# Meng-333/SRADSGAN

Hardware: AMD Instinct MI355X
Metric: training images/sec (216x216, x4) (higher is better)
Workload: dtype f32 (split-bf16 products: 3 bf16 MFMA terms per fp32 multiply, fp32 accumulate)

## Files before the change

sradsgan_amd/csrc/conv_api.hip:

```cpp
#include "conv_internal.h"
#include "conv_dev.h"

using namespace srhip;

namespace srhip {
struct PackEntry {
  const float* w;
  float* packed;
  int cout, cin, kh, kw, mode, fast;
};
__global__ __launch_bounds__(256) void pack_batched_kernel(const PackEntry* __restrict__ tab) {
  const PackEntry e = tab[blockIdx.y];
  const int khkw = e.kh * e.kw;
  if (e.fast) {
    constexpr int LDS_F = 32 * (16 * 9 + 1);
    __shared__ float tile[LDS_F];
    const long total = (long)e.cout * e.cin * khkw;
    const int RO = e.mode == 0 ? 8 : 32;
    const int CI = e.mode == 0 ? (khkw <= 9 ? 64 : 16) : (khkw <= 9 ? 16 : 4);
    const int ld = CI * khkw + 1;
    const int nci = (e.cin + CI - 1) / CI, nco = (e.cout + RO - 1) / RO;
    const int ndst = e.mode == 0 ? e.cout : e.cin, csrc = e.mode == 0 ? e.cin : e.cout;
    const long ndst16 = ((long)ndst + 15) / 16 * 16;
    float* s0 = e.packed;
// ... 194 lines not shown
  }
  if (key == 12) {
    g_flat_blocks = value > 0 ? value : 768;
    return SRHIP_OK;
  }
  if (key == 13) {
    g_flat_abl = value;
    return SRHIP_OK;
  }
  if (key == 14) {
    g_flat_f32_k8 = value;
    return SRHIP_OK;
  }
  if (key == 15) {
    g_patch8 = value;
    return SRHIP_OK;
  }
  if (key == 16) {
    g_patch8_abl = value;
    return SRHIP_OK;
  }
  if (key == 17) {
    g_phase_batch = value;
    return SRHIP_OK;
  }
  if (key == 18) {
    g_headconv_rows = value;
    return SRHIP_OK;
  }
  if (key == 19) {
    g_pool_epi_any = value;
    return SRHIP_OK;
  }
  return SRHIP_ERR_ARG;
}

int srhip_set_conv_math(int mode) {
  SRHIP_REQUIRE(mode == SRHIP_MATH_FP32 || mode == SRHIP_MATH_BF16X3 || mode == SRHIP_MATH_HALF, "set_conv_math: unknown mode");
  g_conv_math = mode;
  return SRHIP_OK;
}
int srhip_get_conv_math(void) { return g_conv_math; }

size_t srhip_packed_elems(int cout, int cin, int kh, int kw, int mode) {
  if (cout <= 0 || cin <= 0 || kh <= 0 || kw <= 0 || (mode != 0 && mode != 1)) return 0;
  const bool fast = mode == 0 ? fast_fwd_ok(cin, cout, kh, kw) : fast_dgrad_ok(cin, cout, kh, kw);
  if (fast)
    return 3 * (size_t)cout * cin * kh * kw + (size_t)fast_tiled_elems(mode == 0 ? cout : cin, mode == 0 ? cin : cout, kh * kw);
  const int csrc = mode == 0 ? cin : cout, cdst = mode == 0 ? cout : cin;
  return (size_t)kh * kw * csrc * legacy_packed_ld(cdst);
}

int srhip_pack_entry_bytes(void) { return (int)sizeof(PackEntry); }

int srhip_packed_is_fast(int cout, int cin, int kh, int kw, int mode) {
  return (mode == 0 ? fast_fwd_ok(cin, cout, kh, kw) : fast_dgrad_ok(cin, cout, kh, kw)) ? 1 : 0;
}

int srhip_pack_weights_batched(const void* entries_dev, int count, void* stream) {
  SRHIP_REQUIRE(entries_dev && count >= 0, "pack_weights_batched: bad argument");
  if (count == 0) return SRHIP_OK;
  hipLaunchKernelGGL(pack_batched_kernel, dim3(32, count), dim3(256), 0, as_stream(stream),
                     static_cast<const PackEntry*>(entries_dev));
  return check_launch("pack_weights_batched");
}

// ... 327 lines not shown
```

sradsgan_amd/csrc/conv_fast.hip:

```cpp
#include "conv_dev.h"

namespace srhip {

int g_fast_ablate = 0;



template <int BM, int BN, int WM, int WN, int BK, int MATH = 0>
__global__ __launch_bounds__(WM* WN * 64) void fast_conv_kernel(const float* __restrict__ src,
                                                                 const float* __restrict__ wt,
                                                                 const float* __restrict__ bias,
                                                                 const float* __restrict__ residual,
                                                                 const float* __restrict__ rowscale,
                                                                 const float* __restrict__ chanscale,
                                                                 const float* __restrict__ actmask,
                                                                 float* __restrict__ dst, FastGeom g, int nblk_m,
                                                                 int nblk_n) {
  constexpr int NT = WM * WN * 64;
  constexpr int WTM = BM / WM, WTN = BN / WN;
  constexpr int TM = WTM / 32, TN = WTN / 32;
  constexpr int LS = BK + 4;
  constexpr int QPR = BK / 4;
  constexpr int RPP = NT / QPR;
  constexpr int AR = (BM + RPP - 1) / RPP, BR = (BN + RPP - 1) / RPP;
// ... 2740 lines not shown
  if (g_conv_math >= 1 && g_wgrad_cfg == 0 && p.bn == 64 && cout % 256 == 0) p.bm = 256;
  if (rowtap == 1) { p.bm = 128; p.bn = 192; }
  if (rowtap == 2) { p.bm = 64; p.bn = 384; }
  const long tiles = (long)cdiv(cout, p.bm) * cdiv(ktot, p.bn);
  const int nchunks = cdiv(P, p.bk);
  const long target = rowtap ? (g_wgrad_cfg >= 100 ? g_wgrad_cfg : 768) : 640;
  long ns = (target + tiles - 1) / tiles;
  const long maxsplit = (nchunks + 15) / 16;
  if (ns > maxsplit) ns = maxsplit;
  if (ns > (tiles <= 2 ? 768 : 256)) ns = tiles <= 2 ? 768 : 256;
  if (ns < 1) ns = 1;
  if (ns >= 8) ns = (ns + 7) / 8 * 8;
  p.chunks_per_split = (int)((nchunks + ns - 1) / ns);
  p.nsplit = cdiv(nchunks, p.chunks_per_split);
  if (p.nsplit >= 8 && p.nsplit % 8 != 0) p.nsplit = (p.nsplit + 7) / 8 * 8;
  return p;
}

static int tail1x1_splits_per_image(int n, int hw) {
  int sp = cdiv(256, n);
  if (sp > cdiv(hw, 64)) sp = cdiv(hw, 64);
  return sp < 1 ? 1 : sp;
}
size_t fast_conv2d_wgrad_workspace(int n, int h, int w, int cin, int cout, int kh, int kw, int stride, int pad) {
  const int ho = (h + 2 * pad - kh) / stride + 1, wo = (w + 2 * pad - kw) / stride + 1;
  const long P = (long)n * ho * wo;
  if (P <= 0) return 0;
  FastWgradPlan p = plan_fast_wgrad(P, cout, kh * kw * cin, rowtap_ok(cin, cout, kh, kw, stride, pad));
  long ns = p.nsplit;
  if (kh == 1 && kw == 1 && cin == 64 && cout == 64 && stride == 1 && pad == 0) {
    const long t = (long)n * tail1x1_splits_per_image(n, h * w);
    if (t > ns) ns = t;
  }
  return (size_t)ns * ((size_t)cout * kh * kw * cin + cout) * sizeof(float);
}

int fast_conv2d_wgrad(const float* x, const float* dy, float* dw, float* db, const float* xrow, const float* xchan,
                      int accumulate, void* workspace, size_t workspace_bytes, int n, int h, int w, int cin, int cout, int kh, int kw, int stride, int pad, int ldx, int ldy,
                      hipStream_t st) {
  SRHIP_REQUIRE(ldx % 4 == 0 && ldy % 4 == 0 && (((uintptr_t)x | (uintptr_t)dy) & 15) == 0,
                "conv2d_wgrad: x/dy must be 16-byte aligned with row strides % 4 == 0");
  WgradGeom g;
  g.N = n; g.H = h; g.W = w; g.C = cin; g.ldx = ldx;
  g.Ho = (h + 2 * pad - kh) / stride + 1;
  g.Wo = (w + 2 * pad - kw) / stride + 1;
  SRHIP_REQUIRE(g.Ho > 0 && g.Wo > 0, "conv2d_wgrad: empty output");
  g.K = cout; g.ldy = ldy; g.KH = kh; g.KW = kw; g.stride = stride; g.pad = pad;
  const long P = (long)n * g.Ho * g.Wo;
  SRHIP_REQUIRE(P < (1L << 31) - 64, "conv2d_wgrad: pixel count overflows int32");
  g.P = (int)P; g.Ktot = kh * kw * cin;
  SRHIP_REQUIRE(bytes_ok((long)n * h * w, ldx, cin, &g.x_bytes) && bytes_ok(P, ldy, cout, &g.dy_bytes),
                "conv2d_wgrad: tensor >= 2 GiB");
  const int rowtap = (!xrow && !xchan) ? rowtap_ok(cin, cout, kh, kw, stride, pad) : 0;
  FastWgradPlan p = plan_fast_wgrad(P, cout, g.Ktot, rowtap);
  g.nsplit = p.nsplit; g.chunks_per_split = p.chunks_per_split;
  const size_t need = (size_t)p.nsplit * ((size_t)cout * g.Ktot + cout) * sizeof(float);
  if (!workspace || workspace_bytes < need) {
    set_error("conv2d_wgrad: workspace %zu bytes < required %zu", workspace_bytes, need);
    return SRHIP_ERR_WORKSPACE;
  }
  float* partial = static_cast<float*>(workspace);
  float* bias_partial = partial + (size_t)p.nsplit * cout * g.Ktot;
  if (xrow && xchan && kh == 1 && kw == 1 && cin == 64 && cout == 64 && stride == 1 && pad == 0 && ldx == 64 && ldy == 64 &&
      g_wgrad_cfg != 8 && g_wgrad_cfg != 6 && n >= 1 &&
      workspace_bytes >= (size_t)n * tail1x1_splits_per_image(n, h * w) * ((size_t)cout * g.Ktot + cout) * sizeof(float)) {
    const int hw = h * w;
    const int sp = tail1x1_splits_per_image(n, hw);
    const int per = (cdiv(hw, sp) + 1) & ~1;
    const int ns = n * sp;
    float* bp = db ? partial + (size_t)ns * cout * g.Ktot : nullptr;
    hipLaunchKernelGGL(wgrad_1x1_scaled_kernel, dim3(ns), dim3(256), 0, st, x, dy, xrow, xchan, partial, bp, hw, per, sp);
    int rc1 = check_launch("wgrad_1x1_scaled");
    if (rc1) return rc1;
    const float* pp[1] = {partial};
    const float* bpp[1] = {bp};
    float* dwp[1] = {dw};
    float* dbp[1] = {db};
    if (launch_reduce4(1, pp, bpp, dwp, dbp, ns, cout, cin, 1, g.Ktot, accumulate, st)) return check_launch("fast_wgrad_reduce4");
    hipLaunchKernelGGL(fast_wgrad_reduce_kernel<4>, dim3(cdiv((long)cout * g.Ktot + (db ? cout : 0), 64)), dim3(256), 0, st, partial, bp, dw, db, ns,
                       cout, cin, 1, g.Ktot, accumulate);
    return check_launch("fast_wgrad_reduce");
  }
  const int blocks = cdiv(cout, p.bm) * cdiv(g.Ktot, p.bn) * p.nsplit;
#define SRHIP_LW(BM_, BN_, WM_, WN_)                                                                              \
  do {                                                                                                            \
// ... 169 lines not shown
```

sradsgan_amd/csrc/conv_internal.h:

```cpp
#pragma once
#include "common.h"

namespace srhip {

int legacy_packed_ld(int cdst);
int legacy_pack_weight(const float* w, float* packed, int cout, int cin, int kh, int kw, int mode, void* stream);
int legacy_conv2d_fwd(const float* x, const float* packed, const float* bias, const float* residual,
                      const float* rowscale, float* y, int n, int h, int w, int cin, int cout, int kh, int kw,
                      int stride, int pad, int ldx, int ldy, int ldr, float slope, int flags, void* stream);
int legacy_conv2d_dgrad(const float* dy, const float* packed, float* dx, int n, int h, int w, int cin, int cout,
                        int kh, int kw, int stride, int pad, int ldy, int ldx, int accumulate, void* stream);
size_t legacy_conv2d_wgrad_workspace(int n, int h, int w, int cin, int cout, int kh, int kw, int stride, int pad);
size_t legacy_conv2d_wgrad_bias_workspace(int n, int h, int w, int cin, int cout, int kh, int kw, int stride, int pad);
int legacy_conv2d_wgrad(const float* x, const float* dy, float* dw, void* workspace, size_t workspace_bytes, int n,
                        int h, int w, int cin, int cout, int kh, int kw, int stride, int pad, int ldx, int ldy,
                        void* stream, float* db = nullptr, float* bias_ws = nullptr, int* bias_done = nullptr,
                        const float* ymask = nullptr, float slope = 0.f);

bool fast_fwd_ok(int cin, int cout, int kh, int kw);
bool fast_dgrad_ok(int cin, int cout, int kh, int kw);
bool fast_wgrad_ok(int cin, int cout, int kh, int kw);
int fast_pack_weight(const float* w, float* packed, int cout, int cin, int kh, int kw, int mode, hipStream_t st);

inline long fast_tiled_elems(int ndst, int csrc, int khkw) { return (long)khkw * csrc * (((long)ndst + 15) / 16 * 16); }
// ... 17 lines not shown
  tp[(q ^ swz) * 8] = h;
  tp[((q + 1) ^ swz) * 8] = l;
}
int fast_conv2d_fwd(const float* x, const float* packed, const float* bias, const float* residual,
                    const float* rowscale, const float* chanscale, float* y, int n, int h, int w, int cin, int cout, int kh, int kw,
                    int stride, int pad, int ldx, int ldy, int ldr, float slope, int flags, hipStream_t st);
int fast_conv2d_dgrad(const float* dy, const float* packed, float* dx, const float* residual, const float* actmask,
                      float slope, int n, int h, int w, int cin, int cout, int kh, int kw, int stride, int pad, int ldy,
                      int ldx, int ldr, int accumulate, hipStream_t st);
int fast_conv2d_fwd_pp(const void* x, int x_pp, const float* packed, const float* bias, void* y, int y_pp, int n, int h, int w, int cin,
                       int cout, int ldx, int ldy, float slope, int flags, hipStream_t st);
int fast_conv2d_dgrad_pp(const void* dy, int dy_pp, const float* packed, void* dx, int dx_pp, const float* residual, const void* actmask,
                         float slope, int n, int h, int w, int cin, int cout, int ldy, int ldx, int ldr, hipStream_t st);
size_t fast_conv2d_wgrad_workspace(int n, int h, int w, int cin, int cout, int kh, int kw, int stride, int pad);
int fast_conv2d_wgrad(const float* x, const float* dy, float* dw, float* db, const float* xrow, const float* xchan,
                      int accumulate, void* workspace, size_t workspace_bytes, int n, int h, int w, int cin, int cout, int kh, int kw, int stride, int pad, int ldx, int ldy,
                      hipStream_t st);

int fast_wgrad_multi_ok(int cin, int cout, int kh, int kw, int stride, int pad);
int fast_wgrad_multi_max(int n, int h, int w, int cin, int cout, int kh, int kw, int stride, int pad);
size_t fast_conv2d_wgrad_multi_workspace(int nprob, int n, int h, int w, int cin, int cout, int kh, int kw, int stride, int pad);
int fast_conv2d_wgrad_multi(int nprob, const float* const* x, const float* const* dy, float* const* dw, float* const* db,
                            int accumulate, void* workspace, size_t workspace_bytes, int n, int h, int w, int cin, int cout,
                            int kh, int kw, int stride, int pad, int ldx, int ldy, hipStream_t st);

int pp_guard(int w);
long pp_plane_pixels(int n, int h, int w);
int pp_from_f32(const float* x, void* pp, int n, int h, int w, int c, int ldx, void* stream);
int pp_to_f32(const void* pp, float* x, int n, int h, int w, int c, int ldx, void* stream);
int flat_wgrad_ok(int n, int h, int w, int cin, int cout);
size_t flat_wgrad_workspace(int nprob, int x_pp, int dy_pp, int n, int h, int w, int cin, int cout);
int flat_wgrad(int nprob, const void* const* x, const void* const* dy, int x_pp, int dy_pp, float* const* dw, float* const* db, int accumulate,
               void* workspace, size_t workspace_bytes, int n, int h, int w, int cin, int cout, int ldf, void* stream);
extern int g_flat_blocks;
extern int g_flat_abl;
extern int g_flat_f32_k8;

size_t colsum_workspace_bytes(long rows, int c);
int colsum_launch(const float* dy, float* db, void* workspace, long rows, int c, int ld, hipStream_t st);

}
```

sradsgan_amd/csrc/conv_wgrad_flat.hip:

```cpp
#include "conv_dev.h"

namespace srhip {

struct FlatGeom {
  int N, H, W, Hp, Wp;
  int C, K;
  int ldf;
  int guard;
  unsigned plane_bytes;
  unsigned pp_bytes, f32_bytes;
  unsigned x_plane_bytes, x_pp_bytes;
  int nchunks, nsplit, cps;
  int Ktot;
};
struct FlatBatch {
  const void* x[4];
  const void* dy[4];
  float* partial[4];
  float* bias_partial[4];
  int nprob, bpp;
};

typedef short s16x4 __attribute__((ext_vector_type(4)));
typedef short s16x8 __attribute__((ext_vector_type(8)));
// ... 303 lines not shown
  }
  if (want_bias) {
    __syncthreads();
    float* bl_ = reinterpret_cast<float*>(lds);
#pragma unroll
    for (int j = 0; j < 8; ++j) bl_[tid * 8 + j] = bsum[j];
    __syncthreads();
    if (tid < BM && m0 + tid < g.K) {
      float s = 0.f;
      if (CFG == 1) {
        const int lgq = tid >> 3, e = tid & 7;
#pragma unroll
        for (int w = 0; w < 4; ++w)
#pragma unroll
          for (int rl = 0; rl < 4; ++rl) {
            const int pgi = (((lgq >> 2) ^ rl) << 2) | (lgq & 3);
            s += bl_[(w * 64 + rl * 16 + pgi) * 8 + e];
          }
      } else {
        const int cq = tid >> 2, e = tid & 3;
#pragma unroll
        for (int w = 0; w < 4; ++w)
#pragma unroll
          for (int rl = 0; rl < 4; ++rl) {
            const int pcq = cq ^ ((((4 * w + rl) >> 1) & 1) << 3);
            s += bl_[(w * 64 + rl * 16 + pcq) * 8 + e];
          }
      }
      bias_partial[(size_t)split * g.K + m0 + tid] = s;
    }
  }
}

template <int CFG, int ABL = 0, int F32 = 0>
__global__ __launch_bounds__(512) void wgrad_flat8_kernel(FlatGeom g, FlatBatch bt) {
  static_assert(CFG == 1 || CFG == 2, "two tile shapes");
  constexpr int TM = 2, TN = 3;
  constexpr int A_B = CFG == 1 ? 16 * 1024 : 4 * 1024;
  constexpr int STAGE_B = CFG == 1 ? 21 * 1024 : 22 * 1024, NSTAGE = 4;
  constexpr int SCRATCH = NSTAGE * STAGE_B;
  __shared__ __attribute__((aligned(1024))) char lds[NSTAGE * STAGE_B + 1024];

  const int tid = threadIdx.x, lane = tid & 63;
  const int wave = __builtin_amdgcn_readfirstlane(tid >> 6);
  const int grp = wave >> 2, w4 = wave & 3;
  const void* xp = bt.x[0];
  const void* dyp = bt.dy[0];
  float* partial = bt.partial[0];
  float* bias_partial = bt.bias_partial[0];
  int bid0 = blockIdx.x;
  if (bt.nprob > 1) {
    const int prob = __builtin_amdgcn_readfirstlane((int)blockIdx.x / bt.bpp);
    bid0 = (int)blockIdx.x - prob * bt.bpp;
    xp = bt.x[prob];
    dyp = bt.dy[prob];
    partial = bt.partial[prob];
    bias_partial = bt.bias_partial[prob];
  }
  constexpr int BMB = CFG == 1 ? 256 : 64, CISB = CFG == 1 ? 64 : 256;
  const int ncs = g.C / CISB, ntn = 3 * ncs, ntm = (g.K + BMB - 1) / BMB;
  int tile_n, tile_m, split;
  {
    const int tps = ntm * ntn, nfull = g.nsplit & ~7;
    int bid = bid0;
    if (bid < nfull * tps) {
      const int j = bid >> 3;
      split = (j / tps) * 8 + (bid & 7);
      bid = j % tps;
    } else {
      bid -= nfull * tps;
      split = nfull + bid / tps;
      bid %= tps;
    }
    tile_n = bid % ntn;
    tile_m = bid / ntn;
  }
  const int kh = tile_n / ncs, cs = tile_n - kh * ncs;
  const int m0 = tile_m * BMB, ci_base = cs * CISB;
  const unsigned lds_base = (unsigned)(size_t)(__attribute__((address_space(3))) char*)lds;
  const int c_begin = split * g.cps;
  const int c_end = min(c_begin + g.cps, g.nchunks);
  const int nk = max(c_end - c_begin, 0);
  const int shiftB = (kh - 1) * g.Wp - 1;

  __amdgpu_buffer_rsrc_t rs_y = __builtin_amdgcn_make_buffer_rsrc(const_cast<void*>(dyp), 0, (F32 && CFG == 2) ? g.f32_bytes : g.pp_bytes, 0x00020000);
  __amdgpu_buffer_rsrc_t rs_x = __builtin_amdgcn_make_buffer_rsrc(const_cast<void*>(xp), 0, (F32 && CFG == 1) ? g.f32_bytes : g.x_pp_bytes, 0x00020000);
  const unsigned y_plane = g.plane_bytes, x_plane = g.x_plane_bytes;
  unsigned d_voff[3], d_dst[3];
  bool d_isx[3];
  {
    auto wide = [&](int piece_in_plane_pair, int nrows, int chan0, int chanC, unsigned, unsigned& voff) {
      const int rr = 4 * piece_in_plane_pair + (lane >> 4);
      const int plane = rr >= nrows ? 1 : 0, r = rr - nrows * plane;
      const int pgl = lane & 15;
      const int lg = (((pgl >> 2) ^ (r & 3)) << 2) | (pgl & 3);
      const int ch = chan0 + lg * 8;
      voff = (rr < 2 * nrows && ch < chanC) ? (unsigned)(r * chanC + ch) * 4u + (unsigned)plane * 16u : F_OOB;
    };
    auto narrow = [&](int piece_in_plane_pair, int nrows, int chan0, int chanC, unsigned, unsigned& voff) {
      const int rr = 8 * piece_in_plane_pair + (lane >> 3);
      const int plane = rr >= nrows ? 1 : 0, r = rr - nrows * plane;
      const int pgl = lane & 7;
      const int lg = (((pgl >> 2) ^ ((r >> 1) & 1)) << 2) | (pgl & 3);
      const int ch = chan0 + lg * 8;
      voff = (rr < 2 * nrows && ch < chanC) ? (unsigned)(r * chanC + ch) * 4u + (unsigned)plane * 16u : F_OOB;
    };
    if (CFG == 1) {
      wide(w4, 16, m0 + 128 * grp, g.K, y_plane, d_voff[0]);
      wide(4 + w4, 16, m0 + 128 * grp, g.K, y_plane, d_voff[1]);
      d_dst[0] = grp * 8192 + w4 * 1024;
      d_dst[1] = grp * 8192 + (4 + w4) * 1024;
      d_isx[0] = d_isx[1] = false;
      narrow(wave < 5 ? wave : 0, 18, ci_base, g.C, x_plane, d_voff[2]);
      if (wave >= 5) d_voff[2] = F_OOB;
      d_dst[2] = wave < 5 ? A_B + wave * 1024 : SCRATCH;
      d_isx[2] = true;
    } else {
      wide(2 * w4, 18, ci_base + 128 * grp, g.C, x_plane, d_voff[0]);
      wide(2 * w4 + 1, 18, ci_base + 128 * grp, g.C, x_plane, d_voff[1]);
      d_dst[0] = A_B + grp * 9216 + (2 * w4) * 1024;
      d_dst[1] = A_B + grp * 9216 + (2 * w4 + 1) * 1024;
      d_isx[0] = d_isx[1] = true;
      if (wave < 4) {
        narrow(wave, 16, m0, g.K, y_plane, d_voff[2]);
        d_dst[2] = wave * 1024;
        d_isx[2] = false;
      } else if (wave < 6) {
        wide(8, 18, ci_base + 128 * (wave - 4), g.C, x_plane, d_voff[2]);
        d_dst[2] = A_B + (wave - 4) * 9216 + 8 * 1024;
        d_isx[2] = true;
      } else {
        d_voff[2] = F_OOB;
        d_dst[2] = SCRATCH;
        d_isx[2] = true;
      }
    }
#pragma unroll
    for (int k = 0; k < 3; ++k) d_dst[k] = __builtin_amdgcn_readfirstlane(lds_base + d_dst[k]);
  }
  const bool f_wave = F32 && wave < (CFG == 1 ? 5 : 4);
  int f_n = 0, f_h = 0, f_w = 0, f_pix = 0;
  unsigned f_choff = 0;
  bool f_live = false;
  if (F32) {
    const int r = 4 * wave + (lane >> 4);
    const int pcq = lane & 15;
    const int cq = pcq ^ (((r >> 1) & 1) << 3);
    const int ch = (CFG == 1 ? ci_base : m0) + cq * 4;
    const int fC = CFG == 1 ? g.C : g.K;
    f_live = f_wave && ch < fC && r < (CFG == 1 ? 18 : 16);
    f_choff = (unsigned)ch * 4u;
    const int per = g.Hp * g.Wp;
    const long q = (long)c_begin * 16 + (CFG == 1 ? shiftB : 0) + r + per;
    const int n1 = (int)(q / per);
    const int rem = (int)(q - (long)n1 * per);
    f_n = n1 - 1;
    f_h = rem / g.Wp;
    f_w = rem - f_h * g.Wp;
    f_pix = (f_n * g.H + f_h) * g.W + f_w;
    if (f_wave) d_dst[2] = __builtin_amdgcn_readfirstlane(lds_base + (CFG == 1 ? A_B : 0) + wave * 1024);
  }
  auto dma_s = [&](unsigned voff, unsigned soff, __amdgpu_buffer_rsrc_t r, unsigned dst) {
    if (ABL & 2) voff = F_OOB;
    asm volatile("s_mov_b32 m0, %3\n\ts_nop 0\n\tbuffer_load_dwordx4 %0, %1, %2 offen lds" ::"v"(voff), "s"(r), "s"(soff), "s"(dst) : "memory");
  };
  const unsigned yC2 = (unsigned)g.K * 4u, xC2 = (unsigned)g.C * 4u;
  auto issue = [&](int c, int stage) {
    const bool live = c < nk;
    const unsigned so_y = (unsigned)(g.guard + (c_begin + c) * 16) * yC2;
    const unsigned so_x = (unsigned)(g.guard + (c_begin + c) * 16 + shiftB) * xC2;
#pragma unroll
    for (int k = 0; k < 3; ++k) {
      const bool isx = d_isx[k];
      const unsigned dst = d_dst[k] == lds_base + SCRATCH ? d_dst[k] : d_dst[k] + stage * STAGE_B;
      if (F32 && k == 2 && f_wave) {
        const bool ok = live && f_live && (unsigned)f_n < (unsigned)g.N && f_h < g.H && f_w < g.W;
        const unsigned vo = ok ? (unsigned)f_pix * (unsigned)g.ldf * 4u + f_choff : F_OOB;
        if (CFG == 1) dma_s(vo, 0u, rs_x, dst);
        else dma_s(vo, 0u, rs_y, dst);
        f_w += 16;
        f_pix += 16;
        while (f_w >= g.Wp) {
          f_w -= g.Wp;
          f_pix -= g.Wp;
          if (++f_h == g.Hp) {
            f_h = 0;
            ++f_n;
          } else {
            f_pix += g.W;
          }
        }
        continue;
      }
      if (isx) dma_s(live ? d_voff[k] : F_OOB, live ? so_x : 0u, rs_x, dst);
      else dma_s(live ? d_voff[k] : F_OOB, live ? so_y : 0u, rs_y, dst);
    }
  };

  constexpr int WN = CFG == 1 ? 2 : 4;
  const int wm = w4 / WN, wn = w4 - wm * WN;
  const int li = lane & 15, g1 = (lane >> 4) & 1, khalf = lane >> 5, l31 = lane & 31;
  const int rq = li >> 2, q4 = li & 3;
  unsigned a_hi[TM], b_hi[TN];
  constexpr int A_LO = CFG == 1 ? 16 * 256 : 16 * 128, B_LO = CFG == 1 ? 18 * 128 : 18 * 256;
  constexpr int A_R4 = (CFG == 1 || F32) ? 1024 : 512, B_R4 = (CFG == 1 && !F32) ? 512 : 1024;
  constexpr bool A_F32 = F32 && CFG == 2, B_F32 = F32 && CFG == 1;
  {
    const int r = 8 * khalf + rq;
#pragma unroll
    for (int t = 0; t < TM; ++t) {
      if (CFG == 1) a_hi[t] = grp * 8192 + r * 256 + (((wm * 2 + t) ^ (r & 3)) << 6) + 32 * g1 + 8 * q4;
      else if (F32) a_hi[t] = r * 256 + (((t * 8 + 4 * g1 + q4) ^ (((r >> 1) & 1) << 3)) << 4) + 8 * (r & 1);
      else a_hi[t] = r * 128 + ((t ^ ((r >> 1) & 1)) << 6) + 32 * g1 + 8 * q4;
    }
#pragma unroll
    for (int u = 0; u < TN; ++u) {
      const int s = r + u;
      if (CFG == 1 && F32) b_hi[u] = A_B + s * 256 + (((wn * 8 + 4 * g1 + q4) ^ (((s >> 1) & 1) << 3)) << 4) + 8 * (s & 1);
      else if (CFG == 1) b_hi[u] = A_B + s * 128 + ((wn ^ ((s >> 1) & 1)) << 6) + 32 * g1 + 8 * q4;
      else b_hi[u] = A_B + grp * 9216 + s * 256 + ((wn ^ (s & 3)) << 6) + 32 * g1 + 8 * q4;
    }
  }
  auto frag = [&](unsigned addr, int r4) {
    bf16x8_t z;
    if (ABL & 4) {
      asm volatile("" : "=v"(z) : "v"(addr));
      return z;
    }
    const s16x4 a = __builtin_amdgcn_ds_read_tr16_b64_v4i16((lds_s16x4_p)(addr));
    const s16x4 b = __builtin_amdgcn_ds_read_tr16_b64_v4i16((lds_s16x4_p)(addr + r4));
    return __builtin_bit_cast(bf16x8_t, __builtin_shufflevector(a, b, 0, 1, 2, 3, 4, 5, 6, 7));
  };
  f32x16 acc[TM][TN];
#pragma unroll
  for (int t = 0; t < TM; ++t)
#pragma unroll
    for (int u = 0; u < TN; ++u)
#pragma unroll
      for (int r = 0; r < 16; ++r) acc[t][u][r] = 0.f;
  const bool want_bias = bias_partial != nullptr;
  const bool bias_wave = CFG == 1 || wave < 4;
  float bsum[8] = {0.f, 0.f, 0.f, 0.f, 0.f, 0.f, 0.f, 0.f};

  auto convert_load = [&](int stage) {
    float4 v = make_float4(0.f, 0.f, 0.f, 0.f);
    if (f_wave) v = __builtin_bit_cast(float4, *reinterpret_cast<const u32x4*>(lds + stage * STAGE_B + (CFG == 1 ? A_B : 0) + wave * 1024 + lane * 16));
    return v;
  };
  auto convert_store = [&](int stage, const float4& v, bool sum_bias) {
    if (!f_wave) return;
    u32x4* slot = reinterpret_cast<u32x4*>(lds + stage * STAGE_B + (CFG == 1 ? A_B : 0) + wave * 1024 + lane * 16);
    typedef __bf16 bf16x2_t __attribute__((ext_vector_type(2)));
    const bf16x2_t h01 = {(__bf16)v.x, (__bf16)v.y}, h23 = {(__bf16)v.z, (__bf16)v.w};
    const unsigned uh01 = __builtin_bit_cast(unsigned, h01), uh23 = __builtin_bit_cast(unsigned, h23);
    const bf16x2_t l01 = {(__bf16)(v.x - __uint_as_float(uh01 << 16)), (__bf16)(v.y - __uint_as_float(uh01 & 0xffff0000u))};
    const bf16x2_t l23 = {(__bf16)(v.z - __uint_as_float(uh23 << 16)), (__bf16)(v.w - __uint_as_float(uh23 & 0xffff0000u))};
    const unsigned ul01 = __builtin_bit_cast(unsigned, l01), ul23 = __builtin_bit_cast(unsigned, l23);
    const bool odd = (lane >> 4) & 1;
    u32x4 o;
    o.x = odd ? ul01 : uh01;
    o.y = odd ? ul23 : uh23;
    o.z = odd ? uh01 : ul01;
    o.w = odd ? uh23 : ul23;
    *slot = o;
    if (CFG == 2 && sum_bias) {
      bsum[0] += v.x; bsum[1] += v.y; bsum[2] += v.z; bsum[3] += v.w;
    }
  };
  auto convert = [&](int stage, bool sum_bias) { convert_store(stage, convert_load(stage), sum_bias); };
  auto bias_chunk = [&](int kc) { return want_bias && (c_begin + kc) % ntn == tile_n; };

  issue(0, 0);
  issue(1, 1);
  issue(2, 2);
  wait_vmcnt<6>();
  if (F32) {
    convert(0, bias_chunk(0));
    asm volatile("s_waitcnt lgkmcnt(0)" ::: "memory");
  }
  __builtin_amdgcn_s_barrier();
  asm volatile("" ::: "memory");
  if (grp == 1) {
    __builtin_amdgcn_s_barrier();
    asm volatile("" ::: "memory");
  }
  for (int kc = 0; kc < nk; ++kc) {
    float4 raw = make_float4(0.f, 0.f, 0.f, 0.f);
    if (F32) {
      wait_vmcnt<3>();
      if (kc + 1 < nk) raw = convert_load((kc + 1) & 3);
    }
    issue(kc + 3, (kc + 3) & 3);
    const unsigned sb = lds_base + (kc & 3) * STAGE_B;
    bf16x8_t ah[TM], al[TM], bh[TN], bl[TN];
#pragma unroll
    for (int t = 0; t < TM; ++t) {
      ah[t] = frag(sb + a_hi[t], A_R4);
      al[t] = frag(sb + (A_F32 ? a_hi[t] ^ 8u : a_hi[t] + A_LO), A_R4);
    }
#pragma unroll
    for (int u = 0; u < TN; ++u) {
      bh[u] = frag(sb + b_hi[u], B_R4);
      bl[u] = frag(sb + (B_F32 ? b_hi[u] ^ 8u : b_hi[u] + B_LO), B_R4);
    }
    if (!A_F32 && want_bias && bias_wave && (c_begin + kc) % ntn == tile_n) {
#pragma unroll
      for (int k = 0; k < (CFG == 1 ? 2 : 1); ++k) {
        const unsigned off = (CFG == 1 ? grp * 8192 + (4 * k + w4) * 1024 : wave * 1024) + lane * 16;
        const u32x4 p = *reinterpret_cast<const u32x4*>(lds + (kc & 3) * STAGE_B + off);
        const unsigned pv[4] = {p.x, p.y, p.z, p.w};
#pragma unroll
        for (int j = 0; j < 4; ++j) {
          bsum[2 * j] += __uint_as_float(pv[j] << 16);
          bsum[2 * j + 1] += __uint_as_float(pv[j] & 0xffff0000u);
        }
      }
    }
    if (F32) {
      if (kc + 1 < nk) convert_store((kc + 1) & 3, raw, bias_chunk(kc + 1));
    } else if (grp == 1) {
      wait_vmcnt<6>();
    }
    asm volatile("s_waitcnt lgkmcnt(0)" ::: "memory");
    __builtin_amdgcn_sched_barrier(0);
    __builtin_amdgcn_s_barrier();
    asm volatile("" ::: "memory");
    __builtin_amdgcn_sched_barrier(0);
    if (!(ABL & 1)) {
      __builtin_amdgcn_s_setprio(1);
#pragma unroll
      for (int i = 0; i < 3 * TM * TN; ++i) {
        const int pr = i / (TM * TN), t = (i % (TM * TN)) / TN, u = i % TN;
        acc[t][u] = __builtin_amdgcn_mfma_f32_32x32x16_bf16(pr == 0 ? al[t] : ah[t], pr == 1 ? bl[u] : bh[u], acc[t][u], 0, 0, 0);
      }
      __builtin_amdgcn_s_setprio(0);
    } else {
#pragma unroll
      for (int t = 0; t < TM; ++t) asm volatile("" ::"v"(ah[t]), "v"(al[t]));
#pragma unroll
      for (int u = 0; u < TN; ++u) asm volatile("" ::"v"(bh[u]), "v"(bl[u]));
    }
    if (!F32 && grp == 0) wait_vmcnt<6>();
    __builtin_amdgcn_sched_barrier(0);
    __builtin_amdgcn_s_barrier();
    asm volatile("" ::: "memory");
    __builtin_amdgcn_sched_barrier(0);
  }
  if (grp == 0) {
    __builtin_amdgcn_s_barrier();
    asm volatile("" ::: "memory");
  }
  wait_vmcnt<0>();

  float* out = partial + (size_t)split * g.K * g.Ktot;
  __syncthreads();
  float* wl = reinterpret_cast<float*>(lds) + wave * (32 * 32);
#pragma unroll
  for (int t = 0; t < TM; ++t) {
#pragma unroll
    for (int u = 0; u < TN; ++u) {
#pragma unroll
      for (int r = 0; r < 16; ++r) wl[((r & 3) + 8 * (r >> 2) + 4 * khalf) * 32 + l31] = acc[t][u][r];
      asm volatile("s_waitcnt lgkmcnt(0)" ::: "memory");
#pragma unroll
      for (int i = 0; i < 4; ++i) {
        const int idx = i * 64 + lane;
        const int row = idx >> 3, cq = idx & 7;
        const float4 v = *reinterpret_cast<const float4*>(wl + row * 32 + cq * 4);
        const int m = m0 + (CFG == 1 ? 128 * grp : 0) + wm * 64 + t * 32 + row;
        const int n = (kh * 3 + u) * g.C + ci_base + (CFG == 2 ? 128 * grp : 0) + wn * 32 + cq * 4;
        if (m < g.K && !(ABL & 8)) *reinterpret_cast<float4*>(out + (size_t)m * g.Ktot + n) = v;
      }
      asm volatile("s_waitcnt lgkmcnt(0)" ::: "memory");
    }
  }
// ... 50 lines not shown
  const long pix = i / c8;
  const int ww = (int)(pix % w);
  const long t = pix / w;
  const int hh = (int)(t % h), nn = (int)(t / h);
  const float4 v0 = *reinterpret_cast<const float4*>(x + pix * ldx + g8 * 8);
  const float4 v1 = *reinterpret_cast<const float4*>(x + pix * ldx + g8 * 8 + 4);
  bf16x8_t hi, lo;
  split_bf16x8(v0, v1, hi, lo);
  const long row = guard + ((long)nn * (h + 1) + hh) * (w + 1) + ww;
  *reinterpret_cast<bf16x8_t*>(pp + row * 2 * c + g8 * 16) = hi;
  *reinterpret_cast<bf16x8_t*>(pp + row * 2 * c + g8 * 16 + 8) = lo;
}
__global__ __launch_bounds__(256) void pp_to_f32_kernel(const __bf16* __restrict__ pp, float* __restrict__ x, int n, int h, int w, int c, int ldx,
                                                        int guard, long plane_elems) {
  const long i = (long)blockIdx.x * 256 + threadIdx.x;
  const int c8 = c >> 3;
  const long total = (long)n * h * w * c8;
  if (i >= total) return;
  const int g8 = (int)(i % c8);
  const long pix = i / c8;
  const int ww = (int)(pix % w);
  const long t = pix / w;
  const int hh = (int)(t % h), nn = (int)(t / h);
  const long row = guard + ((long)nn * (h + 1) + hh) * (w + 1) + ww;
  const bf16x8_t hi = *reinterpret_cast<const bf16x8_t*>(pp + row * 2 * c + g8 * 16);
  const bf16x8_t lo = *reinterpret_cast<const bf16x8_t*>(pp + row * 2 * c + g8 * 16 + 8);
  float o[8];
#pragma unroll
  for (int j = 0; j < 8; ++j) o[j] = (float)hi[j] + (float)lo[j];
  *reinterpret_cast<float4*>(x + pix * ldx + g8 * 8) = make_float4(o[0], o[1], o[2], o[3]);
  *reinterpret_cast<float4*>(x + pix * ldx + g8 * 8 + 4) = make_float4(o[4], o[5], o[6], o[7]);
}

extern int g_conv_math;
int g_flat_abl = 0;
int g_flat_f32_k8 = 1;
int g_flat_blocks = 768;
bool launch_reduce4_shared(int nprob, const float* const* partial, const float* const* bias_partial, float* const* dw, float* const* db,
                           int nsplit, int cout, int cin, int khkw, int ktot, int accumulate, hipStream_t st, int nbias);

int pp_guard(int w) { return ((w + 2) + 15) / 16 * 16; }
long pp_plane_pixels(int n, int h, int w) {
  return (long)pp_guard(w) + (long)n * (h + 1) * (w + 1) + (w + 1) + 48;
}
int pp_from_f32(const float* x, void* pp, int n, int h, int w, int c, int ldx, void* stream) {
  SRHIP_REQUIRE(x && pp && c % 8 == 0 && ldx % 4 == 0 && (((uintptr_t)x | (uintptr_t)pp) & 15) == 0, "pp_from_f32: C %% 8 == 0, 16-byte aligned tensors");
  const long total = (long)n * h * w * (c / 8);
  if (total <= 0) return SRHIP_OK;
  hipLaunchKernelGGL(pp_from_f32_kernel, dim3(cdiv(total, 256)), dim3(256), 0, as_stream(stream), x, static_cast<__bf16*>(pp), n, h, w, c, ldx,
                     pp_guard(w), pp_plane_pixels(n, h, w) * c);
  return check_launch("pp_from_f32");
}
int pp_to_f32(const void* pp, float* x, int n, int h, int w, int c, int ldx, void* stream) {
  SRHIP_REQUIRE(x && pp && c % 8 == 0 && ldx % 4 == 0 && (((uintptr_t)x | (uintptr_t)pp) & 15) == 0, "pp_to_f32: C %% 8 == 0, 16-byte aligned tensors");
  const long total = (long)n * h * w * (c / 8);
  if (total <= 0) return SRHIP_OK;
  hipLaunchKernelGGL(pp_to_f32_kernel, dim3(cdiv(total, 256)), dim3(256), 0, as_stream(stream), static_cast<const __bf16*>(pp), x, n, h, w, c, ldx,
                     pp_guard(w), pp_plane_pixels(n, h, w) * c);
  return check_launch("pp_to_f32");
}

static int num_cus() {
  static int n = 0;
  if (n == 0) {
    int dev = 0;
    if (hipGetDevice(&dev) != hipSuccess || hipDeviceGetAttribute(&n, hipDeviceAttributeMultiprocessorCount, dev) != hipSuccess || n <= 0) n = 256;
  }
  return n;
}
int flat_wgrad_ok(int n, int h, int w, int cin, int cout) {
// ... 100 lines not shown
  const int blocks = bt.bpp * nprob;
  const int cfg = p.cfg;
  if (p.kernel == 8) {
#define SRHIP_F8(ABL_)                                                                                       \
  if (g_flat_abl == ABL_) {                                                                                 \
    if (cfg == 1) hipLaunchKernelGGL((wgrad_flat8_kernel<1, ABL_>), dim3(blocks), dim3(512), 0, st, g, bt);  \
    else hipLaunchKernelGGL((wgrad_flat8_kernel<2, ABL_>), dim3(blocks), dim3(512), 0, st, g, bt);           \
  } else
    SRHIP_F8(1) SRHIP_F8(2) SRHIP_F8(4) SRHIP_F8(8) SRHIP_F8(3) SRHIP_F8(5) SRHIP_F8(6) SRHIP_F8(7) SRHIP_F8(15)
#undef SRHIP_F8
    if (!(x_pp && dy_pp)) {
      if (cfg == 1) hipLaunchKernelGGL((wgrad_flat8_kernel<1, 0, 1>), dim3(blocks), dim3(512), 0, st, g, bt);
      else hipLaunchKernelGGL((wgrad_flat8_kernel<2, 0, 1>), dim3(blocks), dim3(512), 0, st, g, bt);
    } else if (cfg == 1) hipLaunchKernelGGL((wgrad_flat8_kernel<1>), dim3(blocks), dim3(512), 0, st, g, bt);
    else hipLaunchKernelGGL((wgrad_flat8_kernel<2>), dim3(blocks), dim3(512), 0, st, g, bt);
  } else {
#define SRHIP_FA(ABL_)                                                                                   \
  if (g_flat_abl == ABL_) {                                                                             \
    if (cfg == 1) hipLaunchKernelGGL((wgrad_flat_kernel<1, ABL_>), dim3(blocks), dim3(256), 0, st, g, bt); \
    else hipLaunchKernelGGL((wgrad_flat_kernel<2, ABL_>), dim3(blocks), dim3(256), 0, st, g, bt);          \
  } else
    SRHIP_FA(1) SRHIP_FA(2) SRHIP_FA(4) SRHIP_FA(8) SRHIP_FA(16) SRHIP_FA(3) SRHIP_FA(5) SRHIP_FA(6) SRHIP_FA(7) SRHIP_FA(31) SRHIP_FA(23)
#undef SRHIP_FA
    if (cfg == 1) hipLaunchKernelGGL((wgrad_flat_kernel<1>), dim3(blocks), dim3(256), 0, st, g, bt);
    else hipLaunchKernelGGL((wgrad_flat_kernel<2>), dim3(blocks), dim3(256), 0, st, g, bt);
  }
  int rc = check_launch("wgrad_flat");
  if (rc) return rc;
  SRHIP_REQUIRE(launch_reduce4_shared(nprob, bt.partial, bt.bias_partial, dw, db, g.nsplit, cout, cin, 9, g.Ktot, accumulate, st, nbias),
                "conv2d_wgrad_pp: reduce launch refused (alignment)");
  return check_launch("wgrad_flat_reduce");
}

}
```

Measured before the change: 674.5.

## Route stride-2 3x3 weight-gradient convs through phase-split bf16 plane kernel

Adds a path for 3x3 stride-2 pad-1 weight gradients with equal, 256-multiple channel counts. The input is split into four polyphase bf16 hi/lo planes so the existing flat wgrad kernel can treat the strided conv like a stride-1 one. The kernel gains a fourth load slot and a larger LDS stage for the extra input rows. This replaces the generic fast wgrad path for those layers, at the cost of conversion kernels, a larger workspace and a separate bias column-sum.

```diff
diff --git a/sradsgan_amd/csrc/conv_api.hip b/sradsgan_amd/csrc/conv_api.hip
--- a/sradsgan_amd/csrc/conv_api.hip
+++ b/sradsgan_amd/csrc/conv_api.hip
@@ -250,6 +250,10 @@
     g_pool_epi_any = value;
     return SRHIP_OK;
   }
+  if (key == 20) {
+    g_flat_s2 = value;
+    return SRHIP_OK;
+  }
   return SRHIP_ERR_ARG;
 }
 
diff --git a/sradsgan_amd/csrc/conv_fast.hip b/sradsgan_amd/csrc/conv_fast.hip
--- a/sradsgan_amd/csrc/conv_fast.hip
+++ b/sradsgan_amd/csrc/conv_fast.hip
@@ -2796,7 +2796,12 @@
     const long t = (long)n * tail1x1_splits_per_image(n, h * w);
     if (t > ns) ns = t;
   }
-  return (size_t)ns * ((size_t)cout * kh * kw * cin + cout) * sizeof(float);
+  const size_t b = (size_t)ns * ((size_t)cout * kh * kw * cin + cout) * sizeof(float);
+  if (flat_s2_ok(n, h, w, cin, cout, kh, kw, stride, pad)) {
+    const size_t b2 = flat_s2_workspace(1, n, h, w, cin);
+    return b2 > b ? b2 : b;
+  }
+  return b;
 }
 
 int fast_conv2d_wgrad(const float* x, const float* dy, float* dw, float* db, const float* xrow, const float* xchan,
@@ -2815,6 +2820,8 @@
   g.P = (int)P; g.Ktot = kh * kw * cin;
   SRHIP_REQUIRE(bytes_ok((long)n * h * w, ldx, cin, &g.x_bytes) && bytes_ok(P, ldy, cout, &g.dy_bytes),
                 "conv2d_wgrad: tensor >= 2 GiB");
+  if (!xrow && !xchan && flat_s2_ok(n, h, w, cin, cout, kh, kw, stride, pad))
+    return flat_s2_wgrad(1, &x, &dy, &dw, &db, accumulate, workspace, workspace_bytes, n, h, w, cin, ldx, ldy, st);
   const int rowtap = (!xrow && !xchan) ? rowtap_ok(cin, cout, kh, kw, stride, pad) : 0;
   FastWgradPlan p = plan_fast_wgrad(P, cout, g.Ktot, rowtap);
   g.nsplit = p.nsplit; g.chunks_per_split = p.chunks_per_split;
diff --git a/sradsgan_amd/csrc/conv_internal.h b/sradsgan_amd/csrc/conv_internal.h
--- a/sradsgan_amd/csrc/conv_internal.h
+++ b/sradsgan_amd/csrc/conv_internal.h
@@ -73,7 +73,12 @@
 size_t flat_wgrad_workspace(int nprob, int x_pp, int dy_pp, int n, int h, int w, int cin, int cout);
 int flat_wgrad(int nprob, const void* const* x, const void* const* dy, int x_pp, int dy_pp, float* const* dw, float* const* db, int accumulate,
                void* workspace, size_t workspace_bytes, int n, int h, int w, int cin, int cout, int ldf, void* stream);
+int flat_s2_ok(int n, int h, int w, int cin, int cout, int kh, int kw, int stride, int pad);
+size_t flat_s2_workspace(int nprob, int n, int h, int w, int cin);
+int flat_s2_wgrad(int nprob, const float* const* x, const float* const* dy, float* const* dw, float* const* db, int accumulate,
+                  void* workspace, size_t workspace_bytes, int n, int h, int w, int c, int ldx, int ldy, hipStream_t st);
 extern int g_flat_blocks;
+extern int g_flat_s2;
 extern int g_flat_abl;
 extern int g_flat_f32_k8;
 
diff --git a/sradsgan_amd/csrc/conv_wgrad_flat.hip b/sradsgan_amd/csrc/conv_wgrad_flat.hip
--- a/sradsgan_amd/csrc/conv_wgrad_flat.hip
+++ b/sradsgan_amd/csrc/conv_wgrad_flat.hip
@@ -359,12 +359,14 @@
   }
 }
 
-template <int CFG, int ABL = 0, int F32 = 0>
+template <int CFG, int ABL = 0, int F32 = 0, int S2 = 0>
 __global__ __launch_bounds__(512) void wgrad_flat8_kernel(FlatGeom g, FlatBatch bt) {
   static_assert(CFG == 1 || CFG == 2, "two tile shapes");
+  static_assert(!S2 || (CFG == 1 && !F32), "stride 2: CFG 1, both operands planes");
   constexpr int TM = 2, TN = 3;
+  constexpr int NSLOT = S2 ? 4 : 3;
   constexpr int A_B = CFG == 1 ? 16 * 1024 : 4 * 1024;
-  constexpr int STAGE_B = CFG == 1 ? 21 * 1024 : 22 * 1024, NSTAGE = 4;
+  constexpr int STAGE_B = S2 ? 25 * 1024 : CFG == 1 ? 21 * 1024 : 22 * 1024, NSTAGE = 4;
   constexpr int SCRATCH = NSTAGE * STAGE_B;
   __shared__ __attribute__((aligned(1024))) char lds[NSTAGE * STAGE_B + 1024];
 
@@ -408,13 +410,13 @@
   const int c_begin = split * g.cps;
   const int c_end = min(c_begin + g.cps, g.nchunks);
   const int nk = max(c_end - c_begin, 0);
-  const int shiftB = (kh - 1) * g.Wp - 1;
+  const int shiftB = S2 ? (kh == 0 ? -g.Wp : 0) - 1 : (kh - 1) * g.Wp - 1;
 
   __amdgpu_buffer_rsrc_t rs_y = __builtin_amdgcn_make_buffer_rsrc(const_cast<void*>(dyp), 0, (F32 && CFG == 2) ? g.f32_bytes : g.pp_bytes, 0x00020000);
   __amdgpu_buffer_rsrc_t rs_x = __builtin_amdgcn_make_buffer_rsrc(const_cast<void*>(xp), 0, (F32 && CFG == 1) ? g.f32_bytes : g.x_pp_bytes, 0x00020000);
   const unsigned y_plane = g.plane_bytes, x_plane = g.x_plane_bytes;
-  unsigned d_voff[3], d_dst[3];
-  bool d_isx[3];
+  unsigned d_voff[NSLOT], d_dst[NSLOT];
+  bool d_isx[NSLOT];
   {
     auto wide = [&](int piece_in_plane_pair, int nrows, int chan0, int chanC, unsigned, unsigned& voff) {
       const int rr = 4 * piece_in_plane_pair + (lane >> 4);
@@ -432,7 +434,31 @@
       const int ch = chan0 + lg * 8;
       voff = (rr < 2 * nrows && ch < chanC) ? (unsigned)(r * chanC + ch) * 4u + (unsigned)plane * 16u : F_OOB;
     };
-    if (CFG == 1) {
+    auto narrow_s2 = [&](int piece, unsigned& voff) {
+      const int rr = 8 * piece + (lane >> 3);
+      const int sub = rr / 18, r = rr - 18 * sub;
+      const int plane = sub & 1, ecol = sub >> 1;
+      const int pgl = lane & 7;
+      const int lg = (((pgl >> 2) ^ ((r >> 1) & 1)) << 2) | (pgl & 3);
+      const int ch = ci_base + lg * 8;
+      const int q = (kh == 1 ? 0 : 2) + (ecol ? 0 : 1);
+      voff = (r < (ecol ? 16 : 17) && ch < g.C)
+                 ? (unsigned)q * x_plane * 2u + (unsigned)((r + ecol) * g.C + ch) * 4u + (unsigned)plane * 16u : F_OOB;
+    };
+    if (CFG == 1 && S2) {
+      wide(w4, 16, m0 + 128 * grp, g.K, y_plane, d_voff[0]);
+      wide(4 + w4, 16, m0 + 128 * grp, g.K, y_plane, d_voff[1]);
+      d_dst[0] = grp * 8192 + w4 * 1024;
+      d_dst[1] = grp * 8192 + (4 + w4) * 1024;
+      d_isx[0] = d_isx[1] = false;
+      narrow_s2(wave, d_voff[2]);
+      d_dst[2] = A_B + wave * 1024;
+      d_isx[2] = true;
+      narrow_s2(8, d_voff[NSLOT - 1]);
+      if (wave != 0) d_voff[NSLOT - 1] = F_OOB;
+      d_dst[NSLOT - 1] = wave == 0 ? A_B + 8 * 1024 : SCRATCH;
+      d_isx[NSLOT - 1] = true;
+    } else if (CFG == 1) {
       wide(w4, 16, m0 + 128 * grp, g.K, y_plane, d_voff[0]);
       wide(4 + w4, 16, m0 + 128 * grp, g.K, y_plane, d_voff[1]);
       d_dst[0] = grp * 8192 + w4 * 1024;
@@ -463,7 +489,7 @@
       }
     }
 #pragma unroll
-    for (int k = 0; k < 3; ++k) d_dst[k] = __builtin_amdgcn_readfirstlane(lds_base + d_dst[k]);
+    for (int k = 0; k < NSLOT; ++k) d_dst[k] = __builtin_amdgcn_readfirstlane(lds_base + d_dst[k]);
   }
   const bool f_wave = F32 && wave < (CFG == 1 ? 5 : 4);
   int f_n = 0, f_h = 0, f_w = 0, f_pix = 0;
@@ -497,7 +523,7 @@
     const unsigned so_y = (unsigned)(g.guard + (c_begin + c) * 16) * yC2;
     const unsigned so_x = (unsigned)(g.guard + (c_begin + c) * 16 + shiftB) * xC2;
 #pragma unroll
-    for (int k = 0; k < 3; ++k) {
+    for (int k = 0; k < NSLOT; ++k) {
       const bool isx = d_isx[k];
       const unsigned dst = d_dst[k] == lds_base + SCRATCH ? d_dst[k] : d_dst[k] + stage * STAGE_B;
       if (F32 && k == 2 && f_wave) {
@@ -542,8 +568,9 @@
     }
 #pragma unroll
     for (int u = 0; u < TN; ++u) {
-      const int s = r + u;
-      if (CFG == 1 && F32) b_hi[u] = A_B + s * 256 + (((wn * 8 + 4 * g1 + q4) ^ (((s >> 1) & 1) << 3)) << 4) + 8 * (s & 1);
+      const int s = S2 ? r + (u == 2 ? 1 : 0) : r + u;
+      if (S2) b_hi[u] = A_B + (u == 1 ? 36 * 128 : 0) + s * 128 + ((wn ^ ((s >> 1) & 1)) << 6) + 32 * g1 + 8 * q4;
+      else if (CFG == 1 && F32) b_hi[u] = A_B + s * 256 + (((wn * 8 + 4 * g1 + q4) ^ (((s >> 1) & 1) << 3)) << 4) + 8 * (s & 1);
       else if (CFG == 1) b_hi[u] = A_B + s * 128 + ((wn ^ ((s >> 1) & 1)) << 6) + 32 * g1 + 8 * q4;
       else b_hi[u] = A_B + grp * 9216 + s * 256 + ((wn ^ (s & 3)) << 6) + 32 * g1 + 8 * q4;
     }
@@ -600,7 +627,7 @@
   issue(0, 0);
   issue(1, 1);
   issue(2, 2);
-  wait_vmcnt<6>();
+  wait_vmcnt<2 * NSLOT>();
   if (F32) {
     convert(0, bias_chunk(0));
     asm volatile("s_waitcnt lgkmcnt(0)" ::: "memory");
@@ -646,7 +673,7 @@
     if (F32) {
       if (kc + 1 < nk) convert_store((kc + 1) & 3, raw, bias_chunk(kc + 1));
     } else if (grp == 1) {
-      wait_vmcnt<6>();
+      wait_vmcnt<2 * NSLOT>();
     }
     asm volatile("s_waitcnt lgkmcnt(0)" ::: "memory");
     __builtin_amdgcn_sched_barrier(0);
@@ -667,7 +694,7 @@
 #pragma unroll
       for (int u = 0; u < TN; ++u) asm volatile("" ::"v"(bh[u]), "v"(bl[u]));
     }
-    if (!F32 && grp == 0) wait_vmcnt<6>();
+    if (!F32 && grp == 0) wait_vmcnt<2 * NSLOT>();
     __builtin_amdgcn_sched_barrier(0);
     __builtin_amdgcn_s_barrier();
     asm volatile("" ::: "memory");
@@ -784,10 +811,40 @@
   *reinterpret_cast<float4*>(x + pix * ldx + g8 * 8 + 4) = make_float4(o[4], o[5], o[6], o[7]);
 }
 
+__global__ __launch_bounds__(256) void pp_s2_from_f32_kernel(const float* __restrict__ x, __bf16* __restrict__ pp, int n, int h, int w, int c,
+                                                             int ldx, int ho, int wo, int stride, int nimg, int guard, long ppx) {
+  const long i = (long)blockIdx.x * 256 + threadIdx.x;
+  const int c8 = c >> 3;
+  if (i >= (long)nimg * ppx * c8) return;
+  const int g8 = (int)(i % c8);
+  const long rq = i / c8;
+  const int q = (int)(rq / ppx);
+  const long t = rq - (long)q * ppx - guard;
+  const int wp = wo + 1, per = (ho + 1) * wp;
+  u32x4 hi = {0u, 0u, 0u, 0u}, lo = {0u, 0u, 0u, 0u};
+  if (t >= 0 && t < (long)n * per) {
+    const int nn = (int)(t / per);
+    const int rem = (int)(t - (long)nn * per);
+    const int ii = rem / wp, jj = rem - ii * wp;
+    const int hh = stride * ii + (q >> 1), ww = stride * jj + (q & 1);
+    if (ii < ho && jj < wo && hh < h && ww < w) {
+      const float* src = x + (((long)nn * h + hh) * w + ww) * ldx + g8 * 8;
+      bf16x8_t bh, bl;
+      split_bf16x8(*reinterpret_cast<const float4*>(src), *reinterpret_cast<const float4*>(src + 4), bh, bl);
+      hi = __builtin_bit_cast(u32x4, bh);
+      lo = __builtin_bit_cast(u32x4, bl);
+    }
+  }
+  u32x4* dst = reinterpret_cast<u32x4*>(pp + rq * 2 * c + g8 * 16);
+  dst[0] = hi;
+  dst[1] = lo;
+}
+
 extern int g_conv_math;
 int g_flat_abl = 0;
 int g_flat_f32_k8 = 1;
 int g_flat_blocks = 768;
+int g_flat_s2 = 1;
 bool launch_reduce4_shared(int nprob, const float* const* partial, const float* const* bias_partial, float* const* dw, float* const* db,
                            int nsplit, int cout, int cin, int khkw, int ktot, int accumulate, hipStream_t st, int nbias);
 
@@ -954,4 +1011,101 @@
   return check_launch("wgrad_flat_reduce");
 }
 
-}
+static long s2_ho(int h) { return (h - 1) / 2 + 1; }
+static bool flat_s2_shape(int n, int h, int w, int cin, int cout) {
+  if (cin != cout || cout % 256 != 0 || n <= 0 || h < 2 || w < 2) return false;
+  const long ppx = pp_plane_pixels(n, (int)s2_ho(h), (int)s2_ho(w));
+  return 4L * ppx * cin * 4L < (1L << 31) && (long)n * h * w * cin * 4L < (1L << 31);
+}
+int flat_s2_ok(int n, int h, int w, int cin, int cout, int kh, int kw, int stride, int pad) {
+  return g_conv_math == 1 && g_flat_s2 && kh == 3 && kw == 3 && stride == 2 && pad == 1 && flat_s2_shape(n, h, w, cin, cout) ? 1 : 0;
+}
+struct S2Layout {
+  int ho, wo;
+  long ppx;
+  size_t dy_b, x_b, part_b;
+  size_t bias_b, colsum_b;
+  FlatPlan p;
+  int nchunks;
+};
+static S2Layout s2_layout(int nprob, int n, int h, int w, int c) {
+  S2Layout L;
+  L.ho = (int)s2_ho(h);
+  L.wo = (int)s2_ho(w);
+  L.ppx = pp_plane_pixels(n, L.ho, L.wo);
+  L.nchunks = cdiv((long)n * (L.ho + 1) * (L.wo + 1), 16);
+  L.p = flat_plan(1, 1, c, c, L.nchunks, nprob);
+  L.dy_b = ((size_t)L.ppx * c * 4 + 255) & ~(size_t)255;
+  L.x_b = ((size_t)4 * L.ppx * c * 4 + 255) & ~(size_t)255;
+  L.part_b = ((size_t)nprob * L.p.nsplit * (size_t)c * 9 * c * sizeof(float) + 255) & ~(size_t)255;
+  L.bias_b = ((size_t)nprob * c * sizeof(float) + 255) & ~(size_t)255;
+  L.colsum_b = (colsum_workspace_bytes((long)n * L.ho * L.wo, c) + 255) & ~(size_t)255;
+  return L;
+}
+size_t flat_s2_workspace(int nprob, int n, int h, int w, int cin) {
+  const S2Layout L = s2_layout(nprob, n, h, w, cin);
+  return L.part_b + L.bias_b + L.colsum_b + (size_t)nprob * (L.dy_b + L.x_b);
+}
+int flat_s2_wgrad(int nprob, const float* const* x, const float* const* dy, float* const* dw, float* const* db, int accumulate,
+                  void* workspace, size_t workspace_bytes, int n, int h, int w, int c, int ldx, int ldy, hipStream_t st) {
+  SRHIP_REQUIRE(nprob >= 1 && nprob <= 4, "conv2d_wgrad (stride 2, planes): 1..4 problems per launch");
+  SRHIP_REQUIRE(flat_s2_shape(n, h, w, c, c), "conv2d_wgrad (stride 2, planes): shape not served");
+  SRHIP_REQUIRE(ldx % 4 == 0 && ldy % 4 == 0 && ldx >= c && ldy >= c, "conv2d_wgrad (stride 2, planes): row strides");
+  const S2Layout L = s2_layout(nprob, n, h, w, c);
+  SRHIP_REQUIRE(workspace && workspace_bytes >= flat_s2_workspace(nprob, n, h, w, c), "conv2d_wgrad (stride 2, planes): workspace too small");
+  FlatGeom g;
+  g.N = n; g.H = L.ho; g.W = L.wo; g.Hp = L.ho + 1; g.Wp = L.wo + 1;
+  g.C = c; g.K = c; g.ldf = 0;
+  g.guard = pp_guard(L.wo);
+  g.nchunks = L.nchunks;
+  g.plane_bytes = (unsigned)(L.ppx * c * 2L);
+  g.pp_bytes = 2u * g.plane_bytes;
+  g.x_plane_bytes = g.plane_bytes;
+  g.x_pp_bytes = 8u * g.x_plane_bytes;
+  g.f32_bytes = 0;
+  g.nsplit = L.p.nsplit;
+  g.cps = cdiv(g.nchunks, g.nsplit);
+  g.Ktot = 9 * c;
+  const size_t per = (size_t)g.nsplit * c * g.Ktot;
+  float* bias_rows = reinterpret_cast<float*>(static_cast<char*>(workspace) + L.part_b);
+  void* colsum_ws = static_cast<char*>(workspace) + L.part_b + L.bias_b;
+  char* planes = static_cast<char*>(workspace) + L.part_b + L.bias_b + L.colsum_b;
+  const float* bias_row[4];
+  FlatBatch bt;
+  bt.nprob = nprob;
+  bt.bpp = L.p.tiles * g.nsplit;
+  const int c8 = c / 8;
+  for (int i = 0; i < 4; ++i) {
+    const int k = i < nprob ? i : 0;
+    SRHIP_REQUIRE(x[k] && dy[k] && dw[k] && ((((uintptr_t)x[k]) | ((uintptr_t)dy[k])) & 15) == 0, "conv2d_wgrad (stride 2, planes): null / unaligned tensor");
+    char* ypl = planes + (size_t)k * (L.dy_b + L.x_b);
+    char* xpl = ypl + L.dy_b;
+    if (i == k) {
+      const long ty = L.ppx * c8, tx = 4 * L.ppx * c8;
+      hipLaunchKernelGGL(pp_s2_from_f32_kernel, dim3(cdiv(ty, 256)), dim3(256), 0, st, dy[k], reinterpret_cast<__bf16*>(ypl), n, L.ho, L.wo, c, ldy,
+                         L.ho, L.wo, 1, 1, g.guard, L.ppx);
+      hipLaunchKernelGGL(pp_s2_from_f32_kernel, dim3(cdiv(tx, 256)), dim3(256), 0, st, x[k], reinterpret_cast<__bf16*>(xpl), n, h, w, c, ldx,
+                         L.ho, L.wo, 2, 4, g.guard, L.ppx);
+    }
+    float* part = static_cast<float*>(workspace) + per * k;
+    bt.x[i] = xpl;
+    bt.dy[i] = ypl;
+    bt.partial[i] = part;
+    bt.bias_partial[i] = nullptr;
+    bias_row[i] = (db && db[k]) ? bias_rows + (size_t)k * c : nullptr;
+    if (i == k && bias_row[i]) {
+      const int rc0 = colsum_launch(dy[k], bias_rows + (size_t)k * c, colsum_ws, (long)n * L.ho * L.wo, c, ldy, st);
+      if (rc0) return rc0;
+    }
+  }
+  int rc = check_launch("pp_s2_from_f32");
+  if (rc) return rc;
+  hipLaunchKernelGGL((wgrad_flat8_kernel<1, 0, 0, 1>), dim3(bt.bpp * nprob), dim3(512), 0, st, g, bt);
+  rc = check_launch("wgrad_flat_s2");
+  if (rc) return rc;
+  SRHIP_REQUIRE(launch_reduce4_shared(nprob, bt.partial, bias_row, dw, db, g.nsplit, c, c, 9, g.Ktot, accumulate, st, 1),
+                "conv2d_wgrad (stride 2, planes): reduce launch refused (alignment)");
+  return check_launch("wgrad_flat_s2_reduce");
+}
+
+}
```

Measured after the change: 676.4, median of 6. No clear change (+0.3%).
